# Excalibur-SLE/wave-fenics

Hardware: AMD Instinct MI355X
Metric: dofs/sec stiffness-operator apply, P4 hex box mesh (higher is better)
Workload: dtype f64; 1 GPU; P4 hex box 54^3 cells, 10218313 dofs, stiffness + lumped-mass-inverse apply; degree=4, cells_per_gpu=157464, global_dofs=10218313, parallelism=single, kernel=box

## Files before the change

### include/wavehip.h

```cpp
#ifndef WAVEHIP_H
#define WAVEHIP_H

#include <stddef.h>
#include <stdint.h>

#ifdef __cplusplus
extern "C" {
#endif

typedef enum {
  WF_OK = 0,
  WF_ERR_INVALID = -1,
  WF_ERR_UNSUPPORTED = -2,
  WF_ERR_HIP = -3,
  WF_ERR_NODEVICE = -4,
  WF_ERR_COMM = -5
} wf_status;

typedef struct wf_op wf_op;

const char* wf_last_error(void);
const char* wf_version(void);

int wf_device_count(int* count);
// ... 71 lines not shown
  WF_KERNEL_FORCE_ELEMENTWISE = 4,
  WF_KERNEL_FORCE_MARCH = 5,
  WF_KERNEL_FORCE_MASS_MARCH = 6
} wf_kernel_hint;
typedef struct {
  int kernel;
  int variant;
  int lz;
  int lz0;
  int bx, by, bz;
  int keep_cell_order;
  int orient;
  int geometry;
  int metric;
  int update;
} wf_tuning;
typedef enum {
  WF_GEOMETRY_AUTO = 0,
  WF_GEOMETRY_PER_POINT = 1,
  WF_GEOMETRY_PER_CELL = 2
} wf_geometry_mode;
typedef enum {
  WF_METRIC_AUTO = 0,
  WF_METRIC_NONE = 0,
  WF_METRIC_FULL = 1,
  WF_METRIC_AXES = 2
} wf_metric_mode;
typedef enum {
  WF_UPDATE_AUTO = 0,
  WF_UPDATE_NONE = 0,
// ... 78 lines not shown

typedef struct {
  int kind, degree, num_cells, num_dofs_cell, num_quads, ndofs, structured;
  double flops;
  double alg_bytes;
  size_t device_bytes;
  int items_interior, items_interface;
  int kernel;
  int plan_items, plan_patterns, plan_lz;
  int plan_reoriented;
  double plan_fill;
  int geometry;
  int metric;
  int update;
  int cell_coeff;
} wf_op_info_t;
int wf_op_info(const wf_op* op, wf_op_info_t* info);

int wf_box_run_plan(int ncols, int nz, int resident, int nxcd, double prologue, int lz, int32_t* h_runs, int32_t capacity,
                    int32_t* nruns, double* cost, double* uniform_cost, int32_t* uniform_lz);
int wf_op_replan_runs(wf_op* op, int resident);
int wf_op_set_runs(wf_op* op, const int32_t* h_runs, int32_t nruns);
int wf_op_get_runs(const wf_op* op, int32_t* h_runs, int32_t capacity, int32_t* nruns);
int wf_op_destroy(wf_op* op);

int wf_gather(int32_t N, const int32_t* d_indices, const double* d_in, double* d_out, void* stream);
int wf_scatter_add(int32_t N, const int32_t* d_indices, const double* d_in, double* d_out, void* stream);
int wf_scatter_set(int32_t N, const int32_t* d_indices, const double* d_in, double* d_out, void* stream);
int wf_transform1(int32_t N, const double* d_in, const double* d_detJ, double* d_out, void* stream);

int wf_ordered_slots(int64_t ncells, int nd, int32_t ndofs, const int32_t* h_dofmap, int32_t* h_row_off ,
                     int32_t* h_slot );
int wf_segment_sum_add(int32_t n, const int32_t* d_row_off, const double* d_vals, double* d_y, void* stream);

int wf_tsmm(int layout, int64_t ncells, int K, int N, const double* d_in, const double* d_phi, double* d_out,
            void* stream);

int wf_copy(int64_t n, const double* d_in, double* d_out, void* stream);
// ... 116 lines not shown
```

### include/wavehip.hpp

```cpp
#pragma once

#include <cstdint>
#include <cstdlib>
#include <functional>
#include <map>
#include <memory>
#include <stdexcept>
#include <string>
#include <vector>

#include "wavehip.h"

namespace wavehip {

inline void check(int rc)
{
  if (rc != WF_OK) throw std::runtime_error(std::string("wavehip: ") + wf_last_error());
}

inline int set_device(int rank)
{
  check(wf_set_device(rank));
  return rank;
}
// ... 84 lines not shown
  const std::int32_t* geom_dofmap = nullptr;
};

namespace detail {
class OpBase {
public:
  OpBase() = default;
  OpBase(const OpBase&) = delete;
  OpBase& operator=(const OpBase&) = delete;
  virtual ~OpBase() { wf_op_destroy(_op); }
  std::size_t num_quads() const { return info().num_quads; }
  std::size_t num_cells() const { return info().num_cells; }
  std::size_t num_dofs() const { return info().num_dofs_cell; }
  double flops() const { return info().flops; }
  bool cell_coeff() const { return info().cell_coeff != 0; }

  template <typename Vector>
  void apply(const Vector& x, Vector& y, void* stream = nullptr)
  {
    check(wf_op_apply(_op, x.array().data(), y.mutable_array().data(), stream));
  }
  template <typename Vector>
  void operator()(const Vector& x, Vector& y) { apply(x, y); }
  void apply(const double* d_x, double* d_y, void* stream = nullptr) { check(wf_op_apply(_op, d_x, d_y, stream)); }
  wf_op* handle() const { return _op; }

protected:
  wf_op_info_t info() const
  {
    wf_op_info_t i{};
// ... 288 lines not shown
```

### wave_fenics_amd/__init__.py

```python
from ._lib import lib, check, WavehipError
from .box import BoxMesh, FunctionSpace, IndexMap, create_box, create_functionspace, lattice_numbering, renumber
from .operators import (
    StiffnessOperator, MassOperator, SpectralMassOperator, MassOperatorLumped,
    gather, scatter, transform1, tsmm, tabulate_gll, tabulate_dense, precompute_geometric_data,
    quadrature_1d, tabulate_1d, compute_geometry_rule, hex_cell_geometry, ordered_slots, segment_sum_add, box_run_plan,
)
from . import la
from .medium import Medium
```

### wave_fenics_amd/_lib.py

```python
from __future__ import annotations

import ctypes
import os
from ctypes import POINTER, c_char_p, c_double, c_int, c_int32, c_int64, c_size_t, c_void_p

HERE = os.path.dirname(os.path.abspath(__file__))
LIB_PATH = os.environ.get("WAVEHIP_LIB") or os.path.join(HERE, "libwavehip.so")


class WavehipError(RuntimeError):
    """Mirrors the std::runtime_error the reference throws on device failures
    (common/cuda/array.hpp:15-17, mass.hpp:91-92, utils.hpp:30-34)."""


class Tuning(ctypes.Structure):
    _fields_ = [("kernel", c_int), ("variant", c_int), ("lz", c_int), ("lz0", c_int),
                ("bx", c_int), ("by", c_int), ("bz", c_int), ("keep_cell_order", c_int), ("orient", c_int),
                ("geometry", c_int), ("metric", c_int), ("update", c_int)]


class OpDesc(ctypes.Structure):
    _fields_ = [
        ("kind", c_int), ("degree", c_int), ("ncells", c_int), ("ndofs", c_int),
        ("h_dofmap", POINTER(c_int32)), ("h_perm", POINTER(c_int32)),
        ("h_G", POINTER(c_double)), ("h_detJ", POINTER(c_double)),
        ("nverts", c_int), ("h_xverts", POINTER(c_double)), ("h_geom_dofmap", POINTER(c_int32)),
        ("c0", c_double), ("flags", c_int),
        ("nq1", c_int), ("h_phi1", POINTER(c_double)),
        ("h_qpts1", POINTER(c_double)), ("h_qwts1", POINTER(c_double)),
        ("tuning", POINTER(Tuning)),
        ("h_cell_coeff", POINTER(c_double)),
    ]

# ... 14 lines not shown
        ("h_dofmap", POINTER(c_int32)), ("h_phi", POINTER(c_double)), ("h_weights", POINTER(c_double)),
        ("nverts", c_int), ("h_xverts", POINTER(c_double)), ("h_geom_dofmap", POINTER(c_int32)),
        ("flags", c_int),
        ("h_cell_coeff", POINTER(c_double)),
    ]


class OpInfo(ctypes.Structure):
    _fields_ = [
        ("kind", c_int), ("degree", c_int), ("num_cells", c_int), ("num_dofs_cell", c_int),
        ("num_quads", c_int), ("ndofs", c_int), ("structured", c_int),
        ("flops", c_double), ("alg_bytes", c_double), ("device_bytes", c_size_t),
        ("items_interior", c_int), ("items_interface", c_int),
        ("kernel", c_int), ("plan_items", c_int), ("plan_patterns", c_int), ("plan_lz", c_int),
        ("plan_reoriented", c_int), ("plan_fill", c_double), ("geometry", c_int), ("metric", c_int),
        ("update", c_int), ("cell_coeff", c_int),
    ]


class UpdaterDesc(ctypes.Structure):
    _fields_ = [
        ("ndofs", c_int),
        ("num_send_neighbors", c_int), ("send_neighbors", POINTER(c_int)),
        ("send_offsets", POINTER(c_int32)), ("send_indices", POINTER(c_int32)),
        ("num_recv_neighbors", c_int), ("recv_neighbors", POINTER(c_int)),
        ("recv_offsets", POINTER(c_int32)), ("ghost_positions", POINTER(c_int32)),
        ("flags", c_int),
    ]


MATVEC_FN = ctypes.CFUNCTYPE(c_int, c_void_p, c_void_p, c_void_p, c_void_p)
# ... 51 lines not shown
                                       POINTER(c_void_p)]),
    "wf_op_create_box_coeff": (c_int, [c_int, c_int, c_int, c_int, c_int, _dp, c_double, _dp, c_int, POINTER(Tuning),
                                       POINTER(c_void_p)]),
    "wf_op_set_ghost_dofs": (c_int, [c_void_p, _ip, c_int32]),
    "wf_op_create_dense_simplex": (c_int, [POINTER(DenseDesc), POINTER(c_void_p)]),
    "wf_op_create_dense_simplex_mass": (c_int, [POINTER(DenseMassDesc), POINTER(c_void_p)]),
    "wf_op_apply": (c_int, [c_void_p, c_void_p, c_void_p, c_void_p]),
    "wf_op_set_ghost_faces": (c_int, [c_void_p, c_int, c_int, c_int]),
    "wf_op_apply_part": (c_int, [c_void_p, c_void_p, c_void_p, c_int, c_void_p]),
    "wf_op_info": (c_int, [c_void_p, POINTER(OpInfo)]),
    "wf_box_run_plan": (c_int, [c_int, c_int, c_int, c_int, c_double, c_int, POINTER(c_int32), c_int32, POINTER(c_int32),
                                POINTER(c_double), POINTER(c_double), POINTER(c_int32)]),
    "wf_op_replan_runs": (c_int, [c_void_p, c_int]),
    "wf_op_set_runs": (c_int, [c_void_p, POINTER(c_int32), c_int32]),
    "wf_op_get_runs": (c_int, [c_void_p, POINTER(c_int32), c_int32, POINTER(c_int32)]),
    "wf_op_destroy": (c_int, [c_void_p]),
    "wf_gather": (c_int, [c_int32, c_void_p, c_void_p, c_void_p, c_void_p]),
    "wf_scatter_add": (c_int, [c_int32, c_void_p, c_void_p, c_void_p, c_void_p]),
    "wf_scatter_set": (c_int, [c_int32, c_void_p, c_void_p, c_void_p, c_void_p]),
    "wf_transform1": (c_int, [c_int32, c_void_p, c_void_p, c_void_p, c_void_p]),
    "wf_ordered_slots": (c_int, [c_int64, c_int, c_int32, _ip, _ip, _ip]),
    "wf_segment_sum_add": (c_int, [c_int32, c_void_p, c_void_p, c_void_p, c_void_p]),
    "wf_tsmm": (c_int, [c_int, c_int64, c_int, c_int, c_void_p, c_void_p, c_void_p, c_void_p]),
    "wf_copy": (c_int, [c_int64, c_void_p, c_void_p, c_void_p]),
    "wf_fill": (c_int, [c_int64, c_double, c_void_p, c_void_p]),
    "wf_axpy": (c_int, [c_int64, c_double, c_void_p, c_void_p, c_void_p, c_void_p]),
    "wf_scale": (c_int, [c_int64, c_double, c_void_p, c_void_p]),
    "wf_pointwise_div": (c_int, [c_int64, c_void_p, c_void_p, c_void_p, c_void_p]),
    "wf_pointwise_mult_add": (c_int, [c_int64, c_void_p, c_void_p, c_void_p, c_void_p]),
    "wf_dot": (c_int, [c_int64, c_void_p, c_void_p, c_void_p, c_void_p]),
# ... 75 lines not shown
```

### wave_fenics_amd/csrc/common.h

```cpp
#pragma once
#include <hip/hip_runtime.h>

#include <algorithm>
#include <array>
#include <cmath>
#include <cstdint>
#include <cstdio>
#include <cstdlib>
#include <string>
#include <vector>

#include "wavehip.h"

#ifdef WF_DIAG
#define WF_ABLATE_FLAGS(arg) (arg)
#else
#define WF_ABLATE_FLAGS(arg) 0
#endif

namespace wf {

constexpr int kMaxDegree = 7;
constexpr int kMaxN = kMaxDegree + 1;

// ... 79 lines not shown
                             const double* d_D, const DMat& dm, double coeff, const double* d_x,
                             double* d_y, hipStream_t s);
int launch_stiffness_generic_u(int P, int ncells, const int32_t* d_uoff, const int32_t* d_uniq, const uint16_t* d_loc,
                               const double* d_G6blk, const double* d_D, const DMat& dm, double coeff,
                               const double* d_x, double* d_y, hipStream_t s);
int launch_stiffness_box(int P, int nx, int ny, int nz, int bx, int by, int bz, const double* d_G6blk,
                         const double* d_D, const DMat& dm, double coeff, const double* d_x, double* d_y,
                         hipStream_t s);
bool march_variant(int P, int variant, int* bx, int* by);
enum class MarchGeom : int { point = 0, cell = 1, cell_axes = 2 };
int launch_stiffness_march(int P, int variant, MarchGeom geom, int nx, int ny, int nz, int lz, int lz0,
                           const double* d_G6blk, const double* d_Gcell, const double* d_D, const DMat& dm, double coeff,
                           const double* d_x, double* d_y, const int32_t* d_items, int nitems, hipStream_t s);
int march_resident(int P, int variant, MarchGeom geom);
bool march_owner_variant(int P, int variant, int* bx, int* by);
int launch_stiffness_march_owner(int P, int variant, int nx, int ny, int nz, int lz, int lz0, int gbx, int gby,
                                 const double* d_Gcell,
                                 const double* d_D, const DMat& am, double coeff, const double* d_x, double* d_y,
                                 const int32_t* d_items, int nitems, hipStream_t s);
int march_owner_resident(int P, int variant);
struct BoxColumns {
  int nbx, nby;
  int count() const { return nbx * nby; }
};
inline BoxColumns box_columns(int nx, int ny, int bx, int by) { return {(nx + bx - 1) / bx, (ny + by - 1) / by}; }
inline BoxColumns box_owner_columns(int P, int nx, int ny, int bx, int by)
{
  return box_columns(P * nx + 1, P * ny + 1, P * bx, P * by);
}
inline int box_segments(int nz, int lz, int lz0) { return 1 + (std::max(nz - lz0, 0) + lz - 1) / lz; }
struct MarchPlan {
  bool ok = false;
  int BX = 0, BY = 0, lz = 0, nitems = 0, npatterns = 0, tile_size = 0;
  int reoriented = 0, ncomponents = 0;
  double fill = 0.0;
// ... 95 lines not shown
```

### wave_fenics_amd/csrc/op.h

```cpp
#pragma once
#include <functional>
#include <memory>

#include "box_run_plan.h"
#include "device_array.h"

enum class OpKernel : int {
  none = 0,
  box_march,
  box_ksplit,
  box_owner,
  box_block,
  idx_march,
  generic_unique,
  generic_elementwise,
  lumped_unique,
  lumped_elementwise,
  diagonal,
  mass_march,
  mass_column,
  mass_any,
  dense_simplex,
  dense_simplex_mass,
  ordered_stiffness,
// ... 6 lines not shown
  int bx = 1, by = 1, bz = 1;
  int obx = 0, oby = 0;
  int lz = 1;
};

struct wf_op {
  OpKernel kernel = OpKernel::none;
  int kind = 0, P = 0, n = 0, nd = 0, nq = 0, ncells = 0, ndofs = 0;
  int structured = 0, nx = 0, ny = 0, nz = 0;
  BoxChoice box{};
  wf::MarchGeom geom = wf::MarchGeom::point;
  int nq1 = 0;
  int lz0_split = 1;
  double coeff = 0.0;
  int cell_coeff = 0;
  wf::DMat dm{};
  wf::DMat am{};
  wf::DevArray<int32_t> d_dofmap;
  wf::DevArray<double> d_G6blk;
  wf::DevArray<double> d_Gcell;
  wf::DevArray<double> d_detJ;
  wf::DevArray<double> d_D;
  wf::DevArray<double> d_phi1;
  wf::DevArray<double> d_mdiag;
  bool diag_named_only = false;
  wf::DevArray<int32_t> d_uoff, d_uniq;
  wf::DevArray<uint16_t> d_loc;
  int unique_cb = 0;
  int ordered = 0;
  wf::DevArray<int32_t> d_slot, d_row_off;
// ... 79 lines not shown
```

### wave_fenics_amd/csrc/op_apply.hip

```cpp
#include "march_column.h"
#include "op.h"

using namespace wf;

wf_op::~wf_op()
{
  dense_free(dense);
  dense_mass_free(dense_mass);
}

size_t wf::op_device_bytes(const wf_op* op)
{
  size_t total = dense_bytes(op->dense) + dense_mass_bytes(op->dense_mass);
  for (const DevArray<int32_t>* a : {&op->d_dofmap, &op->d_uoff, &op->d_uniq, &op->d_slot, &op->d_row_off, &op->d_items[0],
                                     &op->d_items[1], &op->d_items[2], &op->d_items[3], &op->d_runs, &op->d_item_base, &op->d_item_pattern,
                                     &op->d_item_layers, &op->d_pat_off})
    total += a->bytes();
  for (const DevArray<double>* a : {&op->d_G6blk, &op->d_Gcell, &op->d_detJ, &op->d_D, &op->d_phi1, &op->d_mdiag, &op->d_v})
    total += a->bytes();
  return total + op->d_loc.bytes();
}

namespace {

// ... 120 lines not shown
{
  const double *G6blk = op->d_G6blk.data(), *Gcell = op->d_Gcell.data(), *D = op->d_D.data(), *detJ = op->d_detJ.data(),
               *phi1 = op->d_phi1.data(), *mdiag = op->d_mdiag.data();
  const int32_t *dofmap = op->d_dofmap.data(), *uoff = op->d_uoff.data(), *uniq = op->d_uniq.data(), *slot = op->d_slot.data();
  const uint16_t* loc = op->d_loc.data();
  double* v = op->d_v.data();
  switch (op->kernel) {
    case OpKernel::box_march:
      return launch_stiffness_march(op->P, op->box.variant, op->geom, op->nx, op->ny, op->nz, op->box.lz, lz0, G6blk, Gcell, D,
                                    march_table(op), op->coeff, d_x, d_y, d_items, nitems, s);
    case OpKernel::box_ksplit:
      return launch_stiffness_march_ks_box(op->P, op->box.bx, op->box.by, op->nx, op->ny, op->nz, op->box.lz, lz0, G6blk, D,
                                           op->dm, op->coeff, d_x, d_y, d_items, nitems, s);
    case OpKernel::box_owner:
      if (!d_items && op->d_runs.size())
        return launch_stiffness_march_owner(op->P, op->box.variant, op->nx, op->ny, op->nz, -1, -1, op->box.bx, op->box.by, Gcell,
                                            D, op->am, op->coeff, d_x, d_y, op->d_runs.data(), (int)(op->d_runs.size() / 3), s);
      return launch_stiffness_march_owner(op->P, op->box.variant, op->nx, op->ny, op->nz, op->box.lz, lz0, op->box.bx, op->box.by,
                                          Gcell, D, op->am, op->coeff, d_x, d_y, d_items, nitems, s);
    case OpKernel::box_block:
      return launch_stiffness_box(op->P, op->nx, op->ny, op->nz, op->box.bx, op->box.by, op->box.bz, G6blk, D, op->dm,
                                  op->coeff, d_x, d_y, s);
    case OpKernel::idx_march:
      return launch_stiffness_march_idx(op->P, op->geom, op->plan, op->geom == MarchGeom::point ? G6blk : Gcell, D,
                                        march_table(op), op->coeff, d_x, d_y, d_items, nitems, s);
    case OpKernel::generic_unique:
      return launch_stiffness_generic_u(op->P, op->ncells, uoff, uniq, loc, G6blk, D, op->dm, op->coeff, d_x, d_y, s);
    case OpKernel::generic_elementwise:
      return launch_stiffness_generic(op->P, op->ncells, dofmap, G6blk, D, op->dm, op->coeff, d_x, d_y, s);
    case OpKernel::lumped_unique:
      return launch_mass_lumped_u(op->ncells, op->nd, op->unique_cb, uoff, uniq, loc, detJ, d_x, d_y, s);
    case OpKernel::lumped_elementwise: return launch_mass_lumped((int64_t)op->ncells * op->nd, dofmap, detJ, d_x, d_y, s);
    case OpKernel::diagonal:
      if (op->diag_named_only) return launch_diagonal_named(op->ndofs, mdiag, d_x, d_y, s);
// ... 170 lines not shown
  if (dense && op->cell_coeff) info->alg_bytes += 8.0 * op->ncells;
  if (kernel == WF_KERNEL_CELLS_ORDERED) info->alg_bytes += 20.0 * op->ncells * op->nd + 4.0 * (op->ndofs + 1.0);
  info->device_bytes = op_device_bytes(op);
  info->items_interior = op->nitems[0];
  info->items_interface = op->nitems[1];
  info->kernel = kernel;
  info->plan_items = plan ? op->plan.nitems : 0;
  info->plan_patterns = plan ? op->plan_patterns : 0;
  info->plan_lz = plan ? op->plan.lz : op->d_runs.size() ? op->runs_longest : is_box_march(op->kernel) ? op->box.lz : 0;
  info->plan_reoriented = op->plan_reoriented;
  info->plan_fill = op->plan_fill;
  info->geometry = geometry;
  info->metric = metric;
  info->update = update;
  info->cell_coeff = op->cell_coeff;
  return WF_OK;
}

int wf_op_destroy(wf_op* op)
{
  delete op;
  return WF_OK;
}

}
```

### wave_fenics_amd/csrc/op_create_box.hip

```cpp
#include <cstring>

#include "op.h"

using namespace wf;

namespace {

void default_box_block(int P, const wf_tuning& tun, int* bx, int* by, int* bz)
{
  switch (P) {
    case 1: *bx = 4; *by = 4; *bz = 4; break;
    case 2: *bx = 3; *by = 3; *bz = 3; break;
    case 3: *bx = 4; *by = 2; *bz = 2; break;
    case 4: *bx = 5; *by = 2; *bz = 1; break;
    case 5: *bx = 7; *by = 1; *bz = 1; break;
    case 6: *bx = 5; *by = 1; *bz = 1; break;
    default: *bx = 4; *by = 1; *bz = 1; break;
  }
  if (tun.bx > 0 && tun.by > 0 && tun.bz > 0 && tun.bx * tun.by * tun.bz * (P + 1) * (P + 1) <= 256) {
    *bx = tun.bx;
    *by = tun.by;
    *bz = tun.bz;
  }
}
// ... 63 lines not shown
  if (*geom == MarchGeom::cell_axes) {
    if (tun.update == WF_UPDATE_OWNER || (tun.update == WF_UPDATE_AUTO && P == 4)) {
      if (!march_owner_variant(P, ch->variant, &ch->obx, &ch->oby)) {
        set_error("wf_op_create_box: wf_tuning.variant out of range");
        return WF_ERR_INVALID;
      }
      *kernel = OpKernel::box_owner;
    }
  } else if (tun.update == WF_UPDATE_OWNER) {
    set_error("wf_op_create_box: the owner update needs the separable (axes) form of the marching kernel");
    return WF_ERR_UNSUPPORTED;
  }
  if (!march) return WF_OK;
  const bool owner = *kernel == OpKernel::box_owner;
  const int ncols = owner ? box_owner_columns(P, nx, ny, ch->obx, ch->oby).count() : box_columns(nx, ny, ch->bx, ch->by).count();
  long resident = owner                                 ? march_owner_resident(P, ch->variant)
                  : *kernel == OpKernel::box_march ? march_resident(P, ch->variant, *geom)
                                                        : march_ks_resident(P, ch->bx, ch->by);
  if (resident <= 0) resident = 512;
  ch->lz = box_uniform_lz(ncols, nz, resident, kMarchPrologue, nullptr, nullptr);
  if (tun.lz > 0) ch->lz = tun.lz;
  return WF_OK;
}

int upload_box_cell_geometry(wf_op* op, const std::vector<double>& h_Gc)
{
  const int nx = op->nx, ny = op->ny, nz = op->nz, CB = op->box.bx * op->box.by;
  const BoxColumns cols = box_columns(nx, ny, op->box.bx, op->box.by);
  std::vector<double> blk((size_t)cols.count() * nz * CB * 6, 0.0);
  for (int cz = 0; cz < nz; ++cz)
    for (int cy = 0; cy < ny; ++cy)
      for (int cx = 0; cx < nx; ++cx) {
        const size_t b = (size_t)(cx / op->box.bx) + (size_t)cols.nbx * ((cy / op->box.by) + (size_t)cols.nby * cz);
        const int cl = cx % op->box.bx + op->box.bx * (cy % op->box.by);
        std::memcpy(&blk[(b * CB + cl) * 6], &h_Gc[((size_t)cx + (size_t)nx * (cy + (size_t)ny * cz)) * 6], 6 * sizeof(double));
      }
  return op->d_Gcell.upload(blk);
}

int create_box_ordered(int kind, int P, int nx, int ny, int nz, const double* h_xverts, double c0, const double* h_cell_coeff,
                       int flags, const wf_tuning* tuning, wf_op** out)
{
  const int n = P + 1, nd = n * n * n;
  const size_t NX = (size_t)P * nx + 1, NY = (size_t)P * ny + 1, NZ = (size_t)P * nz + 1;
  const size_t ncells = (size_t)nx * ny * nz;
  std::vector<int32_t> dm(ncells * nd), gd(ncells * 8);
  for (int cz = 0; cz < nz; ++cz)
    for (int cy = 0; cy < ny; ++cy)
      for (int cx = 0; cx < nx; ++cx) {
        const size_t c = (size_t)cx + (size_t)nx * (cy + (size_t)ny * cz);
        const size_t base = (size_t)P * cx + NX * ((size_t)P * cy + NY * ((size_t)P * cz));
// ... 81 lines not shown
  ~EventPair()
  {
    if (e0) (void)hipEventDestroy(e0);
    if (e1) (void)hipEventDestroy(e1);
  }
};

}

int wf::tune_owner_runs(wf_op* op)
{
  op->h_runs.clear();
  op->runs_longest = op->box.lz;
  int rc = op->d_runs.upload(op->h_runs);
  const int ncols = box_owner_columns(op->P, op->nx, op->ny, op->box.obx, op->box.oby).count(), nz = op->nz;
  long resident = march_owner_resident(op->P, op->box.variant);
  if (resident <= 0) resident = 512;
  if (rc != WF_OK || op->P != 4 || op->tun.lz > 0 || (long)ncols * box_segments(nz, op->box.lz, op->box.lz) <= resident) return rc;
  const int lo = std::max(2, (nz + 11) / 12), hi = nz / 4, step = std::max(1, (hi - lo + 16) / 16);
  DevArray<double> vectors;
  if (vectors.alloc(2 * (size_t)op->ndofs) != WF_OK) return (void)hipGetLastError(), WF_OK;
  const double* d_x = vectors.data();
  double* d_y = vectors.data() + op->ndofs;
  WF_HIP_CHECK(hipMemset(vectors.data(), 0, vectors.bytes()));
  EventPair ev;
  WF_HIP_CHECK(hipEventCreate(&ev.e0));
  WF_HIP_CHECK(hipEventCreate(&ev.e1));
  std::vector<int> nsegs = {0};
  for (int nseg = lo; nseg <= hi; nseg += step) nsegs.push_back(nseg);
  std::vector<float> us(nsegs.size(), 1e30f);
  for (int pass = 0; pass < 3; ++pass)
// ... 62 lines not shown
  op->h_runs.assign(h_runs, h_runs + 3 * (size_t)nruns);
  op->runs_longest = nruns ? longest : op->box.lz;
  return op->d_runs.upload(op->h_runs);
}

int wf_op_get_runs(const wf_op* op, int32_t* h_runs, int32_t capacity, int32_t* nruns)
{
  WF_REQUIRE(op && nruns, "wf_op_get_runs: null argument");
  *nruns = (int32_t)(op->h_runs.size() / 3);
  if (op->h_runs.empty() || !h_runs) return WF_OK;
  WF_REQUIRE((size_t)capacity >= op->h_runs.size() / 3, "wf_op_get_runs: h_runs holds fewer than *nruns runs");
  std::memcpy(h_runs, op->h_runs.data(), op->h_runs.size() * sizeof(int32_t));
  return WF_OK;
}

int wf_op_create_box(int kind, int degree, int nx, int ny, int nz, const double* h_xverts, double c0, int flags,
                     wf_op** out)
{
  return wf_op_create_box_coeff(kind, degree, nx, ny, nz, h_xverts, c0, nullptr, flags, nullptr, out);
}

int wf_op_create_box_tuned(int kind, int degree, int nx, int ny, int nz, const double* h_xverts, double c0, int flags,
                           const wf_tuning* tuning, wf_op** out)
{
  return wf_op_create_box_coeff(kind, degree, nx, ny, nz, h_xverts, c0, nullptr, flags, tuning, out);
}

int wf_op_create_box_coeff(int kind, int degree, int nx, int ny, int nz, const double* h_xverts, double c0,
                           const double* h_cell_coeff, int flags, const wf_tuning* tuning, wf_op** out)
{
  WF_REQUIRE(out != nullptr, "wf_op_create_box: null output");
  *out = nullptr;
  const int P = degree;
  if (P < 1 || P > kMaxDegree) {
    set_error("wf_op_create_box: degree must be 1..7 (hexahedron)");
    return WF_ERR_UNSUPPORTED;
  }
  WF_REQUIRE(kind == WF_OP_STIFFNESS || kind == WF_OP_MASS_LUMPED, "wf_op_create_box: kind must be stiffness or lumped mass");
  WF_REQUIRE(!tuning || tuning->kernel != WF_KERNEL_FORCE_MASS_MARCH,
             "wf_op_create_box: WF_KERNEL_FORCE_MASS_MARCH applies to the dense mass only");
  WF_REQUIRE(nx > 0 && ny > 0 && nz > 0 && h_xverts, "wf_op_create_box: bad mesh");
  const size_t NX = (size_t)P * nx + 1, NY = (size_t)P * ny + 1, NZ = (size_t)P * nz + 1;
  WF_REQUIRE(NX * NY * NZ < ((size_t)1 << 31), "wf_op_create_box: dof lattice exceeds int32");
  const int n = P + 1, nd = n * n * n;
  const size_t ncells = (size_t)nx * ny * nz;
  if (int bad = check_cell_coeff(h_cell_coeff, ncells, "wf_op_create_box")) return bad;
  if (flags & WF_FLAG_ORDERED) return create_box_ordered(kind, P, nx, ny, nz, h_xverts, c0, h_cell_coeff, flags, tuning, out);

  OpPtr op = new_op(kind, P, nd, nd, nx * ny * nz, (int)(NX * NY * NZ), c0, tuning);
  op->cell_coeff = h_cell_coeff != nullptr;
  op->nq1 = n;
  op->structured = 1;
  op->nx = nx;
  op->ny = ny;
  op->nz = nz;

// ... 44 lines not shown
```

### wave_fenics_amd/csrc/stiffness_march_owner.hip

```cpp
#include <cstdlib>

#include "march_column.h"
#include "stiffness_core.h"

namespace wf {

#ifndef WF_OWNER_WAVES
#define WF_OWNER_WAVES 3
#endif
#ifndef WF_OWNER_WAVES_HI
#define WF_OWNER_WAVES_HI 2
#endif

template <int P>
constexpr int owner_waves() { return P >= 5 ? WF_OWNER_WAVES_HI : WF_OWNER_WAVES; }

#ifndef WF_OWNER_LANE_EXCHANGE
#define WF_OWNER_LANE_EXCHANGE 1
#endif

template <int P>
constexpr bool owner_lane_exchange() { return WF_OWNER_LANE_EXCHANGE != 0 && P == 4; }

template <int P, int BX, int BY>
// ... 19 lines not shown
template <int CTRL>
__device__ __forceinline__ double dpp_move(double v)
{
  const int lo = __builtin_amdgcn_mov_dpp(__double2loint(v), CTRL, 0xf, 0xf, false);
  const int hi = __builtin_amdgcn_mov_dpp(__double2hiint(v), CTRL, 0xf, 0xf, false);
  return __hiloint2double(hi, lo);
}
__device__ __forceinline__ double add_rounded(double a, double b)
{
#pragma clang fp contract(off)
  return a + b;
}
constexpr int dpp_quad(int a) { return a | a << 2 | a << 4 | a << 6; }
constexpr int dpp_row_ror(int n) { return 0x120 + n; }

template <int P, int BX, int BY>
__global__ __launch_bounds__(256, (owner_waves<P>())) void k_stiffness_owner(
    int nx, int ny, int nz, int lz, int lz0, int gbx, int gby, const double* __restrict__ Gc, const double* __restrict__ dD, DMat am,
    double coeff, const double* __restrict__ x, double* __restrict__ y, const int32_t* __restrict__ items,
    int ablate_arg)
{
  [[maybe_unused]] const int ablate = WF_ABLATE_FLAGS(ablate_arg);
  constexpr int n = P + 1;
  constexpr int LX = P * BX, LY = P * BY, NL = LX * LY;
  constexpr int RX = LX + P + 1, RY = LY + P + 1, RP = RX * RY;
  constexpr int NPF = (P * RP + 255) / 256;
  constexpr int NCP = (RP + 255) / 256;
  constexpr int GCX = BX + 1, GC = GCX * (BY + 1), NG = 3 * GC;
  constexpr int NGL = (NG + 255) / 256;
  static_assert(NL <= 256, "column does not fit a 256-thread workgroup");
  constexpr bool lx = owner_lane_exchange<P>();
// ... 98 lines not shown
    const double x_ar = g0[AR], x_br = g0[BR], x_al = g0[AL], x_bl = g0[BL];
    const double y_ar = g1[AR], y_al = g1[AL], y_br = g1[BR], y_bl = g1[BL];
    const double z_ar = g2[AR], z_al = g2[AL], z_br = g2[BR], z_bl = g2[BL];
    s[0] = cwj * (mj ? x_ar + x_br : x_ar);
    s[1] = mi ? cwj * (mj ? x_al + x_bl : x_al) : 0.0;
    s[2] = cwi * (mi ? y_ar + y_al : y_ar);
    s[3] = mj ? cwi * (mi ? y_br + y_bl : y_br) : 0.0;
    const double za = mi ? z_ar + z_al : z_ar, zb = mi ? z_br + z_bl : z_br;
    s[4] = cwij * (mj ? za + zb : za);
  };

  double xz[2 * P + 1];
  double sc[5], sf[4], spz;
  double yA[P], yB[P];
  {
    double gp[NGL], gcur[NGL];
    load_g(gp, z0 > 0 ? z0 - 1 : z0);
    load_g(gcur, z0);
#pragma unroll
    for (int m = 0; m < P; ++m) {
      const long K = (long)P * z0 - P + m;
      const double v = x[plane * (size_t)(K >= 0 ? K : 0) + yoff];
      xz[m] = K >= 0 ? v : 0.0;
    }
#pragma unroll
    for (int k = 0; k < P; ++k) yA[k] = (ablate & 1) ? 0.0 : y[plane * (size_t)(P * z0 + k) + yoff];
    const double* xb = x + plane * (size_t)(P * z0) + plane;
    double xp0[NCP], xp[NPF];
#pragma unroll
    for (int m = 0; m < NCP; ++m) xp0[m] = (xb - plane)[t + 256 * m < RP && poff[m] >= 0 ? poff[m] : pclamp];
#pragma unroll
    for (int m = 0; m < NPF; ++m) xp[m] = xb[poff[m] >= 0 ? poff[m] : pclamp];
#pragma unroll
    for (int m = 0; m < NCP; ++m) {
      const int pos = t + 256 * m;
      Ux[tile_or_dump<RP>(m, pos, 0, (P + 1) * RP, t)] = (pos < RP && poff[m] >= 0) ? xp0[m] : 0.0;
    }
#pragma unroll
    for (int m = 0; m < NPF; ++m) {
      const int pos = t + 256 * m;
      Ux[tile_or_dump<P * RP>(m, pos, RP, (P + 1) * RP, t)] = poff[m] >= 0 ? xp[m] : 0.0;
    }
    store_g(gp);
    __syncthreads();
    double sp[5];
    scales(sp);
    if (z0 == 0)
#pragma unroll
      for (int q = 0; q < 5; ++q) sp[q] = 0.0;
    __syncthreads();
    store_g(gcur);
    __syncthreads();
    scales(sc);
#pragma unroll
    for (int q = 0; q < 4; ++q) sf[q] = lx ? add_rounded(sc[q], sp[q]) : sc[q] + sp[q];
    spz = sp[4];
#pragma unroll
    for (int m = 0; m <= P; ++m) xz[P + m] = Ux[m * RP + rown + cown];
  }
  [[maybe_unused]] double zpc = 0.0;
  if constexpr (lx) {
#pragma unroll
    for (int a = 0; a < n; ++a) zpc += arow(P, a) * xz[a];
  }

  if (ablate & 16) {
    double u = zpc + spz;
#pragma unroll
// ... 56 lines not shown
    double* dst = y + plane * K + yoff;
    if (ablate & 1) {
      if (v == 1.2345e300) *dst = v;
    } else if (own) {
      *dst = v;
    }
  };

  auto layer = [&](auto hn_tag, double (&ycur)[P], double (&ynext)[P], int kz) {
    constexpr bool has_next = decltype(hn_tag)::value;
    [[maybe_unused]] double xn[NPF], gn[NGL];
    if constexpr (has_next) {
      const double* xb = x + plane * (size_t)(P * (kz + 1) + 1);
#pragma unroll
      for (int m = 0; m < NPF; ++m) xn[m] = xb[poff[m] >= 0 ? poff[m] : pclamp];
      load_g(gn, kz + 1);
#pragma unroll
      for (int k = 0; k < P; ++k) ynext[k] = (ablate & 1) ? 0.0 : y[plane * (size_t)(P * (kz + 1) + k) + yoff];
    }

#pragma unroll
    for (int k = 0; k < P; ++k) {
      double zc = 0.0;
#pragma unroll
      for (int a = 0; a < n; ++a) zc += arow(k, a) * xz[P + a];
      double v;
      if (k == 0) {
        double zp = 0.0;
        if constexpr (lx) {
          zp = zpc;
        } else {
// ... 18 lines not shown
      for (int m = 0; m < NCP; ++m) {
        const int pos = t + 256 * m;
        xcp[m] = pos < RP ? Ux[P * RP + pos] : 0.0;
      }
      __syncthreads();
#pragma unroll
      for (int m = 0; m < NCP; ++m) {
        const int pos = t + 256 * m;
        Ux[tile_or_dump<RP>(m, pos, 0, (P + 1) * RP, t)] = xcp[m];
      }
#pragma unroll
      for (int m = 0; m < NPF; ++m) {
        const int pos = t + 256 * m;
        Ux[tile_or_dump<P * RP>(m, pos, RP, (P + 1) * RP, t)] = poff[m] >= 0 ? xn[m] : 0.0;
      }
      store_g(gn);
      __syncthreads();
#pragma unroll
      for (int m = 0; m <= P; ++m) xz[m] = xz[m + P];
#pragma unroll
      for (int m = 1; m <= P; ++m) xz[P + m] = Ux[m * RP + rown + cown];
      double sn[5];
      scales(sn);
#pragma unroll
      for (int q = 0; q < 4; ++q) sf[q] = lx ? add_rounded(sn[q], sc[q]) : sn[q] + sc[q];
      spz = sc[4];
#pragma unroll
      for (int q = 0; q < 5; ++q) sc[q] = sn[q];
    }
  };

  for (int kz = z0; kz < z1; kz += 2) {
    if (kz + 1 < z1) {
      layer(On{}, yA, yB, kz);
      if (kz + 2 < z1)
        layer(On{}, yB, yA, kz + 1);
      else
        layer(Off{}, yB, yA, kz + 1);
    } else {
      layer(Off{}, yA, yB, kz);
    }
  }

  if (z1 == nz) {
    double zp = 0.0;
#pragma unroll
    for (int a = 0; a < n; ++a) zp += arow(P, a) * xz[P + a];
    const double v = wk[0] * xy_terms(P, sc[0], sc[1], sc[2], sc[3]) + zp * sc[4];
    const size_t K = (size_t)P * nz;
    const double y0 = (ablate & 1) ? 0.0 : y[plane * K + yoff];
    store_y(K, y0 + v);
  }
}

template <int P, int BX, int BY>
static int launch_owner_t(int nx, int ny, int nz, int lz, int lz0, int gbx, int gby, const double* d_Gcell, const double* d_D,
                          const DMat& am, double coeff, const double* d_x, double* d_y, const int32_t* d_items, int nitems,
                          hipStream_t s)
{
  const int nwg = d_items ? nitems : box_owner_columns(P, nx, ny, BX, BY).count() * box_segments(nz, lz, lz0);
  if (nwg == 0) return WF_OK;
  hipLaunchKernelGGL((k_stiffness_owner<P, BX, BY>), dim3((unsigned)nwg), dim3(256), 0, s, nx, ny, nz, lz, lz0, gbx, gby, d_Gcell,
                     d_D, am, coeff, d_x, d_y, d_items, ablate_flags());
  return launch_status("stiffness_march (owner)");
}

#define WF_OWNER_SHAPES(X)                                                                                \
  X(1, 0, 16, 16) X(1, 1, 32, 8) X(1, 2, 8, 32)                                          \
  X(2, 0, 8, 8) X(2, 1, 16, 4) X(2, 2, 4, 16)                                            \
  X(3, 0, 5, 5) X(3, 1, 7, 3) X(3, 2, 3, 7)                                  \
  X(4, 0, 4, 4) X(4, 1, 8, 2) X(4, 2, 2, 8)      \
  X(5, 0, 3, 3) X(5, 1, 5, 2) X(5, 2, 2, 5)           \
  X(6, 0, 3, 2) X(6, 1, 7, 1) X(6, 2, 2, 3)           \
  X(7, 0, 2, 2) X(7, 1, 5, 1) X(7, 2, 1, 5)

bool march_owner_variant(int P, int variant, int* bx, int* by)
{
#define X(PP, V, BXX, BYY) \
  if (P == PP && variant == V) return *bx = BXX, *by = BYY, true;
  WF_OWNER_SHAPES(X)
#undef X
  return false;
}

int launch_stiffness_march_owner(int P, int variant, int nx, int ny, int nz, int lz, int lz0, int gbx, int gby,
                                 const double* d_Gcell,
                                 const double* d_D, const DMat& am, double coeff, const double* d_x, double* d_y,
                                 const int32_t* d_items, int nitems, hipStream_t s)
{
  if ((size_t)nx * ny * nz == 0) return WF_OK;
#define X(PP, V, BXX, BYY) \
  if (P == PP && variant == V) return launch_owner_t<PP, BXX, BYY>(nx, ny, nz, lz, lz0, gbx, gby, d_Gcell, d_D, am, coeff, d_x, d_y, d_items, nitems, s);
  WF_OWNER_SHAPES(X)
#undef X
  set_error("stiffness_march (owner): unsupported degree/variant");
  return WF_ERR_UNSUPPORTED;
}

int march_owner_resident(int P, int variant)
{
#define X(PP, V, BXX, BYY) \
  if (P == PP && variant == V) return resident_workgroups(k_stiffness_owner<PP, BXX, BYY>);
  WF_OWNER_SHAPES(X)
#undef X
  return 0;
}

}
```

### wave_fenics_amd/operators.py

```python
from __future__ import annotations

import ctypes
from ctypes import POINTER, c_double, c_int32, c_void_p

import numpy as np

from . import _lib
from ._lib import OpDesc, OpInfo, check, lib
from .box import FunctionSpace


def _ptr(t) -> int:
    if isinstance(t, int):
        return t
    return int(t.data_ptr())


def _stream(t=None) -> int:
    try:
        import torch
        if t is not None and hasattr(t, "is_cuda") and t.is_cuda:
            return int(torch.cuda.current_stream(t.device).cuda_stream)
    except ImportError:
        pass
# ... 68 lines not shown
    detJ = np.zeros((mesh.ncells, nq))
    check(lib().wf_geometry_hex_rule(mesh.ncells, x.shape[0], _dp(x), _ip(gd), pts.size, _dp(pts), _dp(wts),
                                     int(use_fabs), int(clamp), _dp(G), _dp(detJ)))
    return G, detJ


def hex_cell_geometry(mesh, p: int, use_fabs: bool = True, clamp: bool = True):
    x = np.ascontiguousarray(mesh.x, dtype=np.float64)
    gd = np.ascontiguousarray(mesh.geom_dofmap, dtype=np.int32)
    ncells = gd.size // 8
    Gc = np.zeros((ncells, 6))
    bad, reason = ctypes.c_int64(-1), ctypes.c_int(0)
    check(lib().wf_geometry_hex_cell(p, ncells, x.shape[0], _dp(x), _ip(gd), int(use_fabs), int(clamp), _dp(Gc),
                                     ctypes.byref(bad), ctypes.byref(reason)))
    return Gc, int(bad.value), int(reason.value)


def precompute_geometric_data(mesh, p: int, use_fabs: bool = True, clamp: bool = True, want_G: bool = True):
    nq = (p + 1) ** 3
    x = np.ascontiguousarray(mesh.x, dtype=np.float64)
    gd = np.ascontiguousarray(mesh.geom_dofmap, dtype=np.int32)
    G = np.zeros((mesh.ncells, nq, 3, 3)) if want_G else None
    detJ = np.zeros((mesh.ncells, nq))
    check(lib().wf_geometry_hex(p, mesh.ncells, x.shape[0], _dp(x), _ip(gd), int(use_fabs), int(clamp),
                                _dp(G), _dp(detJ)))
    return G, detJ


def make_tuning(tuning) -> "_lib.Tuning | None":
    if tuning is None:
# ... 6 lines not shown
    t = _lib.Tuning()
    k = tuning.get("kernel", 0)
    t.kernel = names[k] if isinstance(k, str) else int(k)
    t.variant = int(tuning.get("variant", -1)) + 1
    t.lz = int(tuning.get("lz", 0))
    t.lz0 = int(tuning.get("lz0", 0))
    t.bx, t.by, t.bz = (int(v) for v in tuning.get("block", (0, 0, 0)))
    t.keep_cell_order = int(bool(tuning.get("keep_cell_order", False)))
    t.orient = int(tuning.get("orient", 0))
    g = tuning.get("geometry", 0)
    t.geometry = GEOMETRY_MODES[g] if isinstance(g, str) else int(g)
    m = tuning.get("metric", 0)
    t.metric = METRIC_MODES[m] if isinstance(m, str) else int(m)
    u = tuning.get("update", 0)
    t.update = UPDATE_MODES[u] if isinstance(u, str) else int(u)
    return t


GEOMETRY_MODES = {"auto": 0, "per_point": 1, "per_cell": 2}
METRIC_MODES = {"auto": 0, "full": 1, "axes": 2}
UPDATE_MODES = {"auto": 0, "atomic": 1, "owner": 2}
KERNEL_NAMES = {0: "none", 1: "march_box", 2: "march_idx", 3: "batch_unique", 4: "box_block", 5: "diagonal",
                6: "mass_dense_any", 7: "dense_simplex", 8: "elementwise", 9: "cells_ordered",
                10: "dense_simplex_mass"}


class _Operator:
    _kind = None

    def __init__(self):
# ... 10 lines not shown
        self._keep = ()
        self._info()

    def _create_box(self, kind: int, p: int, mesh, c0: float, flags: int, tuning=None, cell_coeff=None):
        nx, ny, nz = mesh.n
        x = np.ascontiguousarray(mesh.x, dtype=np.float64)
        a = _cell_coeff(cell_coeff, nx * ny * nz)
        t = make_tuning(tuning)
        check(lib().wf_op_create_box_coeff(kind, p, nx, ny, nz, _dp(x), float(c0), _dp(a), flags,
                                           ctypes.byref(t) if t is not None else None, ctypes.byref(self._h)))
        self._info()

    @property
    def cell_coeff(self) -> bool:
        return bool(self.info.cell_coeff)

    @property
    def kernel(self) -> str:
        return KERNEL_NAMES.get(self.info.kernel, "?")

    @property
    def geometry(self) -> str:
        return {1: "per_point", 2: "per_cell"}.get(self.info.geometry, "none")

    @property
    def metric(self) -> str:
        return {1: "full", 2: "axes"}.get(self.info.metric, "none")

    @property
    def update(self) -> str:
# ... 245 lines not shown
```

Baseline: 120.2 billion dofs/s.

## Specialize owner march kernel for z-invariant cell geometry

At box-operator creation the blocked per-cell geometry is compared layer by layer with an exact memcmp. When every z layer matches, a templated variant of the owner march stiffness kernel runs instead. It loads the geometry once, skips the per-layer geometry load, LDS store and scale recomputation, and reuses the current scales as the previous-layer scales. The z segment length is also re-planned from the new kernel's residency, and a tuning flag lets users disable the path. The cost is a second kernel instantiation and a host-side scan at setup.

```diff
diff --git a/include/wavehip.h b/include/wavehip.h
--- a/include/wavehip.h
+++ b/include/wavehip.h
@@ -109,6 +109,7 @@
   int geometry;
   int metric;
   int update;
+  int z_invariant;
 } wf_tuning;
 typedef enum {
   WF_GEOMETRY_AUTO = 0,
@@ -217,6 +218,7 @@
   int metric;
   int update;
   int cell_coeff;
+  int z_invariant;
 } wf_op_info_t;
 int wf_op_info(const wf_op* op, wf_op_info_t* info);
 
@@ -225,6 +227,8 @@
 int wf_op_replan_runs(wf_op* op, int resident);
 int wf_op_set_runs(wf_op* op, const int32_t* h_runs, int32_t nruns);
 int wf_op_get_runs(const wf_op* op, int32_t* h_runs, int32_t capacity, int32_t* nruns);
+int wf_box_z_invariant(int degree, int nx, int ny, int nz, const double* h_xverts, const double* h_cell_coeff, int flags,
+                       int bx, int by, int* z_invariant);
 int wf_op_destroy(wf_op* op);
 
 int wf_gather(int32_t N, const int32_t* d_indices, const double* d_in, double* d_out, void* stream);
diff --git a/include/wavehip.hpp b/include/wavehip.hpp
--- a/include/wavehip.hpp
+++ b/include/wavehip.hpp
@@ -122,6 +122,7 @@
   std::size_t num_dofs() const { return info().num_dofs_cell; }
   double flops() const { return info().flops; }
   bool cell_coeff() const { return info().cell_coeff != 0; }
+  bool z_invariant() const { return info().z_invariant != 0; }
 
   template <typename Vector>
   void apply(const Vector& x, Vector& y, void* stream = nullptr)
diff --git a/wave_fenics_amd/__init__.py b/wave_fenics_amd/__init__.py
--- a/wave_fenics_amd/__init__.py
+++ b/wave_fenics_amd/__init__.py
@@ -4,6 +4,7 @@
     StiffnessOperator, MassOperator, SpectralMassOperator, MassOperatorLumped,
     gather, scatter, transform1, tsmm, tabulate_gll, tabulate_dense, precompute_geometric_data,
     quadrature_1d, tabulate_1d, compute_geometry_rule, hex_cell_geometry, ordered_slots, segment_sum_add, box_run_plan,
+    box_z_invariant,
 )
 from . import la
 from .medium import Medium
diff --git a/wave_fenics_amd/_lib.py b/wave_fenics_amd/_lib.py
--- a/wave_fenics_amd/_lib.py
+++ b/wave_fenics_amd/_lib.py
@@ -16,7 +16,7 @@
 class Tuning(ctypes.Structure):
     _fields_ = [("kernel", c_int), ("variant", c_int), ("lz", c_int), ("lz0", c_int),
                 ("bx", c_int), ("by", c_int), ("bz", c_int), ("keep_cell_order", c_int), ("orient", c_int),
-                ("geometry", c_int), ("metric", c_int), ("update", c_int)]
+                ("geometry", c_int), ("metric", c_int), ("update", c_int), ("z_invariant", c_int)]
 
 
 class OpDesc(ctypes.Structure):
@@ -61,7 +61,7 @@
         ("items_interior", c_int), ("items_interface", c_int),
         ("kernel", c_int), ("plan_items", c_int), ("plan_patterns", c_int), ("plan_lz", c_int),
         ("plan_reoriented", c_int), ("plan_fill", c_double), ("geometry", c_int), ("metric", c_int),
-        ("update", c_int), ("cell_coeff", c_int),
+        ("update", c_int), ("cell_coeff", c_int), ("z_invariant", c_int),
     ]
 
 
@@ -143,6 +143,7 @@
     "wf_op_replan_runs": (c_int, [c_void_p, c_int]),
     "wf_op_set_runs": (c_int, [c_void_p, POINTER(c_int32), c_int32]),
     "wf_op_get_runs": (c_int, [c_void_p, POINTER(c_int32), c_int32, POINTER(c_int32)]),
+    "wf_box_z_invariant": (c_int, [c_int, c_int, c_int, c_int, _dp, _dp, c_int, c_int, c_int, POINTER(c_int)]),
     "wf_op_destroy": (c_int, [c_void_p]),
     "wf_gather": (c_int, [c_int32, c_void_p, c_void_p, c_void_p, c_void_p]),
     "wf_scatter_add": (c_int, [c_int32, c_void_p, c_void_p, c_void_p, c_void_p]),
diff --git a/wave_fenics_amd/csrc/common.h b/wave_fenics_amd/csrc/common.h
--- a/wave_fenics_amd/csrc/common.h
+++ b/wave_fenics_amd/csrc/common.h
@@ -117,11 +117,11 @@
                            const double* d_x, double* d_y, const int32_t* d_items, int nitems, hipStream_t s);
 int march_resident(int P, int variant, MarchGeom geom);
 bool march_owner_variant(int P, int variant, int* bx, int* by);
-int launch_stiffness_march_owner(int P, int variant, int nx, int ny, int nz, int lz, int lz0, int gbx, int gby,
-                                 const double* d_Gcell,
+int launch_stiffness_march_owner(int P, int variant, bool z_invariant, int nx, int ny, int nz, int lz, int lz0, int gbx,
+                                 int gby, const double* d_Gcell,
                                  const double* d_D, const DMat& am, double coeff, const double* d_x, double* d_y,
                                  const int32_t* d_items, int nitems, hipStream_t s);
-int march_owner_resident(int P, int variant);
+int march_owner_resident(int P, int variant, bool z_invariant);
 struct BoxColumns {
   int nbx, nby;
   int count() const { return nbx * nby; }
diff --git a/wave_fenics_amd/csrc/op.h b/wave_fenics_amd/csrc/op.h
--- a/wave_fenics_amd/csrc/op.h
+++ b/wave_fenics_amd/csrc/op.h
@@ -44,6 +44,7 @@
   int lz0_split = 1;
   double coeff = 0.0;
   int cell_coeff = 0;
+  int z_invariant = 0;
   wf::DMat dm{};
   wf::DMat am{};
   wf::DevArray<int32_t> d_dofmap;
diff --git a/wave_fenics_amd/csrc/op_apply.hip b/wave_fenics_amd/csrc/op_apply.hip
--- a/wave_fenics_amd/csrc/op_apply.hip
+++ b/wave_fenics_amd/csrc/op_apply.hip
@@ -158,10 +158,11 @@
                                            op->dm, op->coeff, d_x, d_y, d_items, nitems, s);
     case OpKernel::box_owner:
       if (!d_items && op->d_runs.size())
-        return launch_stiffness_march_owner(op->P, op->box.variant, op->nx, op->ny, op->nz, -1, -1, op->box.bx, op->box.by, Gcell,
-                                            D, op->am, op->coeff, d_x, d_y, op->d_runs.data(), (int)(op->d_runs.size() / 3), s);
-      return launch_stiffness_march_owner(op->P, op->box.variant, op->nx, op->ny, op->nz, op->box.lz, lz0, op->box.bx, op->box.by,
-                                          Gcell, D, op->am, op->coeff, d_x, d_y, d_items, nitems, s);
+        return launch_stiffness_march_owner(op->P, op->box.variant, op->z_invariant != 0, op->nx, op->ny, op->nz, -1, -1, op->box.bx,
+                                            op->box.by, Gcell, D, op->am, op->coeff, d_x, d_y, op->d_runs.data(),
+                                            (int)(op->d_runs.size() / 3), s);
+      return launch_stiffness_march_owner(op->P, op->box.variant, op->z_invariant != 0, op->nx, op->ny, op->nz, op->box.lz, lz0,
+                                          op->box.bx, op->box.by, Gcell, D, op->am, op->coeff, d_x, d_y, d_items, nitems, s);
     case OpKernel::box_block:
       return launch_stiffness_box(op->P, op->nx, op->ny, op->nz, op->box.bx, op->box.by, op->box.bz, G6blk, D, op->dm,
                                   op->coeff, d_x, d_y, s);
@@ -362,6 +363,7 @@
   info->metric = metric;
   info->update = update;
   info->cell_coeff = op->cell_coeff;
+  info->z_invariant = op->z_invariant;
   return WF_OK;
 }
 
diff --git a/wave_fenics_amd/csrc/op_create_box.hip b/wave_fenics_amd/csrc/op_create_box.hip
--- a/wave_fenics_amd/csrc/op_create_box.hip
+++ b/wave_fenics_amd/csrc/op_create_box.hip
@@ -101,7 +101,7 @@
   if (!march) return WF_OK;
   const bool owner = *kernel == OpKernel::box_owner;
   const int ncols = owner ? box_owner_columns(P, nx, ny, ch->obx, ch->oby).count() : box_columns(nx, ny, ch->bx, ch->by).count();
-  long resident = owner                                 ? march_owner_resident(P, ch->variant)
+  long resident = owner                                 ? march_owner_resident(P, ch->variant, false)
                   : *kernel == OpKernel::box_march ? march_resident(P, ch->variant, *geom)
                                                         : march_ks_resident(P, ch->bx, ch->by);
   if (resident <= 0) resident = 512;
@@ -110,18 +110,39 @@
   return WF_OK;
 }
 
-int upload_box_cell_geometry(wf_op* op, const std::vector<double>& h_Gc)
-{
-  const int nx = op->nx, ny = op->ny, nz = op->nz, CB = op->box.bx * op->box.by;
-  const BoxColumns cols = box_columns(nx, ny, op->box.bx, op->box.by);
+std::vector<double> block_cell_geometry(int nx, int ny, int nz, int bx, int by, const std::vector<double>& h_Gc)
+{
+  const int CB = bx * by;
+  const BoxColumns cols = box_columns(nx, ny, bx, by);
   std::vector<double> blk((size_t)cols.count() * nz * CB * 6, 0.0);
   for (int cz = 0; cz < nz; ++cz)
     for (int cy = 0; cy < ny; ++cy)
       for (int cx = 0; cx < nx; ++cx) {
-        const size_t b = (size_t)(cx / op->box.bx) + (size_t)cols.nbx * ((cy / op->box.by) + (size_t)cols.nby * cz);
-        const int cl = cx % op->box.bx + op->box.bx * (cy % op->box.by);
+        const size_t b = (size_t)(cx / bx) + (size_t)cols.nbx * ((cy / by) + (size_t)cols.nby * cz);
+        const int cl = cx % bx + bx * (cy % by);
         std::memcpy(&blk[(b * CB + cl) * 6], &h_Gc[((size_t)cx + (size_t)nx * (cy + (size_t)ny * cz)) * 6], 6 * sizeof(double));
       }
+  return blk;
+}
+
+bool cell_layers_equal(const std::vector<double>& blk, int nz)
+{
+  const size_t layer = blk.size() / (size_t)nz;
+  for (int cz = 1; cz < nz; ++cz)
+    if (std::memcmp(&blk[layer * cz], blk.data(), layer * sizeof(double)) != 0) return false;
+  return true;
+}
+
+int upload_box_cell_geometry(wf_op* op, const std::vector<double>& h_Gc)
+{
+  const std::vector<double> blk = block_cell_geometry(op->nx, op->ny, op->nz, op->box.bx, op->box.by, h_Gc);
+  op->z_invariant = op->kernel == OpKernel::box_owner && op->tun.z_invariant == 0 && cell_layers_equal(blk, op->nz);
+  if (op->z_invariant && op->tun.lz <= 0) {
+    const long general = march_owner_resident(op->P, op->box.variant, false), resident = march_owner_resident(op->P, op->box.variant, true);
+    if (resident > 0 && resident != general)
+      op->box.lz = box_uniform_lz(box_owner_columns(op->P, op->nx, op->ny, op->box.obx, op->box.oby).count(), op->nz, resident,
+                                  kMarchPrologue, nullptr, nullptr);
+  }
   return op->d_Gcell.upload(blk);
 }
 
@@ -233,7 +254,7 @@
   op->runs_longest = op->box.lz;
   int rc = op->d_runs.upload(op->h_runs);
   const int ncols = box_owner_columns(op->P, op->nx, op->ny, op->box.obx, op->box.oby).count(), nz = op->nz;
-  long resident = march_owner_resident(op->P, op->box.variant);
+  long resident = march_owner_resident(op->P, op->box.variant, op->z_invariant != 0);
   if (resident <= 0) resident = 512;
   if (rc != WF_OK || op->P != 4 || op->tun.lz > 0 || (long)ncols * box_segments(nz, op->box.lz, op->box.lz) <= resident) return rc;
   const int lo = std::max(2, (nz + 11) / 12), hi = nz / 4, step = std::max(1, (hi - lo + 16) / 16);
@@ -326,6 +347,22 @@
   return WF_OK;
 }
 
+int wf_box_z_invariant(int degree, int nx, int ny, int nz, const double* h_xverts, const double* h_cell_coeff, int flags,
+                       int bx, int by, int* z_invariant)
+{
+  WF_REQUIRE(degree >= 1 && degree <= kMaxDegree && nx > 0 && ny > 0 && nz > 0 && bx > 0 && by > 0 && h_xverts && z_invariant,
+             "wf_box_z_invariant: bad argument");
+  const size_t ncells = (size_t)nx * ny * nz;
+  if (int bad = check_cell_coeff(h_cell_coeff, ncells, "wf_box_z_invariant")) return bad;
+  std::vector<double> h_Gc;
+  WF_REQUIRE(box_cell_geometry(degree, nx, ny, nz, h_xverts, fabs_flag(flags), clamp_flag(flags), h_Gc),
+             "wf_box_z_invariant: the mesh has no per-cell geometry (a cell is not affine, or the -1/0/1 clamp takes effect)");
+  if (h_cell_coeff)
+    for (size_t e = 0; e < h_Gc.size(); ++e) h_Gc[e] *= h_cell_coeff[e / 6];
+  *z_invariant = cell_layers_equal(block_cell_geometry(nx, ny, nz, bx, by, h_Gc), nz) ? 1 : 0;
+  return WF_OK;
+}
+
 int wf_op_create_box(int kind, int degree, int nx, int ny, int nz, const double* h_xverts, double c0, int flags,
                      wf_op** out)
 {
@@ -352,6 +389,7 @@
   WF_REQUIRE(!tuning || tuning->kernel != WF_KERNEL_FORCE_MASS_MARCH,
              "wf_op_create_box: WF_KERNEL_FORCE_MASS_MARCH applies to the dense mass only");
   WF_REQUIRE(nx > 0 && ny > 0 && nz > 0 && h_xverts, "wf_op_create_box: bad mesh");
+  WF_REQUIRE(!tuning || tuning->z_invariant == 0 || tuning->z_invariant == 1, "wf_op_create_box: wf_tuning.z_invariant out of range");
   const size_t NX = (size_t)P * nx + 1, NY = (size_t)P * ny + 1, NZ = (size_t)P * nz + 1;
   WF_REQUIRE(NX * NY * NZ < ((size_t)1 << 31), "wf_op_create_box: dof lattice exceeds int32");
   const int n = P + 1, nd = n * n * n;
diff --git a/wave_fenics_amd/csrc/stiffness_march_owner.hip b/wave_fenics_amd/csrc/stiffness_march_owner.hip
--- a/wave_fenics_amd/csrc/stiffness_march_owner.hip
+++ b/wave_fenics_amd/csrc/stiffness_march_owner.hip
@@ -57,7 +57,7 @@
 constexpr int dpp_quad(int a) { return a | a << 2 | a << 4 | a << 6; }
 constexpr int dpp_row_ror(int n) { return 0x120 + n; }
 
-template <int P, int BX, int BY>
+template <int P, int BX, int BY, bool ZI>
 __global__ __launch_bounds__(256, (owner_waves<P>())) void k_stiffness_owner(
     int nx, int ny, int nz, int lz, int lz0, int gbx, int gby, const double* __restrict__ Gc, const double* __restrict__ dD, DMat am,
     double coeff, const double* __restrict__ x, double* __restrict__ y, const int32_t* __restrict__ items,
@@ -186,9 +186,10 @@
   double sc[5], sf[4], spz;
   double yA[P], yB[P];
   {
-    double gp[NGL], gcur[NGL];
-    load_g(gp, z0 > 0 ? z0 - 1 : z0);
-    load_g(gcur, z0);
+    [[maybe_unused]] double gp[NGL];
+    double gcur[NGL];
+    if constexpr (!ZI) load_g(gp, z0 > 0 ? z0 - 1 : z0);
+    load_g(gcur, ZI ? 0 : z0);
 #pragma unroll
     for (int m = 0; m < P; ++m) {
       const long K = (long)P * z0 - P + m;
@@ -213,17 +214,25 @@
       const int pos = t + 256 * m;
       Ux[tile_or_dump<P * RP>(m, pos, RP, (P + 1) * RP, t)] = poff[m] >= 0 ? xp[m] : 0.0;
     }
-    store_g(gp);
-    __syncthreads();
     double sp[5];
-    scales(sp);
-    if (z0 == 0)
-#pragma unroll
-      for (int q = 0; q < 5; ++q) sp[q] = 0.0;
-    __syncthreads();
-    store_g(gcur);
-    __syncthreads();
-    scales(sc);
+    if constexpr (ZI) {
+      store_g(gcur);
+      __syncthreads();
+      scales(sc);
+#pragma unroll
+      for (int q = 0; q < 5; ++q) sp[q] = z0 == 0 ? 0.0 : sc[q];
+    } else {
+      store_g(gp);
+      __syncthreads();
+      scales(sp);
+      if (z0 == 0)
+#pragma unroll
+        for (int q = 0; q < 5; ++q) sp[q] = 0.0;
+      __syncthreads();
+      store_g(gcur);
+      __syncthreads();
+      scales(sc);
+    }
 #pragma unroll
     for (int q = 0; q < 4; ++q) sf[q] = lx ? add_rounded(sc[q], sp[q]) : sc[q] + sp[q];
     spz = sp[4];
@@ -310,7 +319,8 @@
       const double* xb = x + plane * (size_t)(P * (kz + 1) + 1);
 #pragma unroll
       for (int m = 0; m < NPF; ++m) xn[m] = xb[poff[m] >= 0 ? poff[m] : pclamp];
-      load_g(gn, kz + 1);
+      if constexpr (!ZI)
+        if (!(ablate & 32)) load_g(gn, kz + 1);
 #pragma unroll
       for (int k = 0; k < P; ++k) ynext[k] = (ablate & 1) ? 0.0 : y[plane * (size_t)(P * (kz + 1) + k) + yoff];
     }
@@ -359,19 +369,31 @@
         const int pos = t + 256 * m;
         Ux[tile_or_dump<P * RP>(m, pos, RP, (P + 1) * RP, t)] = poff[m] >= 0 ? xn[m] : 0.0;
       }
-      store_g(gn);
+      if constexpr (!ZI)
+        if (!(ablate & 32)) store_g(gn);
       __syncthreads();
 #pragma unroll
       for (int m = 0; m <= P; ++m) xz[m] = xz[m + P];
 #pragma unroll
       for (int m = 1; m <= P; ++m) xz[P + m] = Ux[m * RP + rown + cown];
-      double sn[5];
-      scales(sn);
-#pragma unroll
-      for (int q = 0; q < 4; ++q) sf[q] = lx ? add_rounded(sn[q], sc[q]) : sn[q] + sc[q];
-      spz = sc[4];
-#pragma unroll
-      for (int q = 0; q < 5; ++q) sc[q] = sn[q];
+      if constexpr (ZI) {
+#pragma unroll
+        for (int q = 0; q < 4; ++q) sf[q] = lx ? add_rounded(sc[q], sc[q]) : sc[q] + sc[q];
+        spz = sc[4];
+      } else {
+        double sn[5];
+        if (ablate & 32) {
+#pragma unroll
+          for (int q = 0; q < 5; ++q) sn[q] = sc[q];
+        } else {
+          scales(sn);
+        }
+#pragma unroll
+        for (int q = 0; q < 4; ++q) sf[q] = lx ? add_rounded(sn[q], sc[q]) : sn[q] + sc[q];
+        spz = sc[4];
+#pragma unroll
+        for (int q = 0; q < 5; ++q) sc[q] = sn[q];
+      }
     }
   };
 
@@ -398,14 +420,14 @@
   }
 }
 
-template <int P, int BX, int BY>
+template <int P, int BX, int BY, bool ZI>
 static int launch_owner_t(int nx, int ny, int nz, int lz, int lz0, int gbx, int gby, const double* d_Gcell, const double* d_D,
                           const DMat& am, double coeff, const double* d_x, double* d_y, const int32_t* d_items, int nitems,
                           hipStream_t s)
 {
   const int nwg = d_items ? nitems : box_owner_columns(P, nx, ny, BX, BY).count() * box_segments(nz, lz, lz0);
   if (nwg == 0) return WF_OK;
-  hipLaunchKernelGGL((k_stiffness_owner<P, BX, BY>), dim3((unsigned)nwg), dim3(256), 0, s, nx, ny, nz, lz, lz0, gbx, gby, d_Gcell,
+  hipLaunchKernelGGL((k_stiffness_owner<P, BX, BY, ZI>), dim3((unsigned)nwg), dim3(256), 0, s, nx, ny, nz, lz, lz0, gbx, gby, d_Gcell,
                      d_D, am, coeff, d_x, d_y, d_items, ablate_flags());
   return launch_status("stiffness_march (owner)");
 }
@@ -428,24 +450,29 @@
   return false;
 }
 
-int launch_stiffness_march_owner(int P, int variant, int nx, int ny, int nz, int lz, int lz0, int gbx, int gby,
-                                 const double* d_Gcell,
+int launch_stiffness_march_owner(int P, int variant, bool z_invariant, int nx, int ny, int nz, int lz, int lz0, int gbx,
+                                 int gby, const double* d_Gcell,
                                  const double* d_D, const DMat& am, double coeff, const double* d_x, double* d_y,
                                  const int32_t* d_items, int nitems, hipStream_t s)
 {
   if ((size_t)nx * ny * nz == 0) return WF_OK;
-#define X(PP, V, BXX, BYY) \
-  if (P == PP && variant == V) return launch_owner_t<PP, BXX, BYY>(nx, ny, nz, lz, lz0, gbx, gby, d_Gcell, d_D, am, coeff, d_x, d_y, d_items, nitems, s);
+#define X(PP, V, BXX, BYY)                                                                                             \
+  if (P == PP && variant == V)                                                                                         \
+    return z_invariant ? launch_owner_t<PP, BXX, BYY, true>(nx, ny, nz, lz, lz0, gbx, gby, d_Gcell, d_D, am, coeff, d_x, \
+                                                            d_y, d_items, nitems, s)                                   \
+                       : launch_owner_t<PP, BXX, BYY, false>(nx, ny, nz, lz, lz0, gbx, gby, d_Gcell, d_D, am, coeff,   \
+                                                             d_x, d_y, d_items, nitems, s);
   WF_OWNER_SHAPES(X)
 #undef X
   set_error("stiffness_march (owner): unsupported degree/variant");
   return WF_ERR_UNSUPPORTED;
 }
 
-int march_owner_resident(int P, int variant)
-{
-#define X(PP, V, BXX, BYY) \
-  if (P == PP && variant == V) return resident_workgroups(k_stiffness_owner<PP, BXX, BYY>);
+int march_owner_resident(int P, int variant, bool z_invariant)
+{
+#define X(PP, V, BXX, BYY)     \
+  if (P == PP && variant == V) \
+    return z_invariant ? resident_workgroups(k_stiffness_owner<PP, BXX, BYY, true>) : resident_workgroups(k_stiffness_owner<PP, BXX, BYY, false>);
   WF_OWNER_SHAPES(X)
 #undef X
   return 0;
diff --git a/wave_fenics_amd/operators.py b/wave_fenics_amd/operators.py
--- a/wave_fenics_amd/operators.py
+++ b/wave_fenics_amd/operators.py
@@ -106,6 +106,15 @@
     check(lib().wf_geometry_hex_cell(p, ncells, x.shape[0], _dp(x), _ip(gd), int(use_fabs), int(clamp), _dp(Gc),
                                      ctypes.byref(bad), ctypes.byref(reason)))
     return Gc, int(bad.value), int(reason.value)
+
+
+def box_z_invariant(mesh, p: int, cell_coeff=None, block=(1, 1), flags: int = 0) -> bool:
+    nx, ny, nz = mesh.n
+    x = np.ascontiguousarray(mesh.x, dtype=np.float64)
+    a = _cell_coeff(cell_coeff, nx * ny * nz)
+    out = ctypes.c_int(0)
+    check(lib().wf_box_z_invariant(int(p), nx, ny, nz, _dp(x), _dp(a), int(flags), int(block[0]), int(block[1]), ctypes.byref(out)))
+    return bool(out.value)
 
 
 def precompute_geometric_data(mesh, p: int, use_fabs: bool = True, clamp: bool = True, want_G: bool = True):
@@ -142,6 +151,7 @@
     t.metric = METRIC_MODES[m] if isinstance(m, str) else int(m)
     u = tuning.get("update", 0)
     t.update = UPDATE_MODES[u] if isinstance(u, str) else int(u)
+    t.z_invariant = int(tuning.get("z_invariant", 0))
     return t
 
 
@@ -182,6 +192,10 @@
     @property
     def cell_coeff(self) -> bool:
         return bool(self.info.cell_coeff)
+
+    @property
+    def z_invariant(self) -> int:
+        return int(self.info.z_invariant)
 
     @property
     def kernel(self) -> str:
```

After: 119.9 billion dofs/s. Within noise of the previous version (-0.3%).
